# davidbau/rewriting

Hardware: NVIDIA H100
Metric: StyleGAN2-256 images/sec (higher is better)
Workload: dtype bf16x3 (3-term split bf16 operands, fp32 accumulate; fp32 in/out)

## Files before the change

### rewriting_b200/csrc/conv_tc.cu

```cuda
#include <cstdlib>
#include <cstring>

#include "rw_common.cuh"
#include "rw_kernels.h"

namespace rw {

namespace {

constexpr int BM = 128;
constexpr int BK = 32;
constexpr int MMA_K = 16;
constexpr int kStages = 7;
constexpr int kNumThreads = 384;
constexpr int kTmaWarp = 8;
constexpr uint32_t kProducerRegs = 40;
constexpr uint32_t kConsumerRegs = 232;
constexpr int kCluster = 2;
constexpr int kChunkKB = 16;

template <int BN>
struct ConvSmem {
  static constexpr int kABytes = BM * BK * 2;
  static constexpr int kBBytes = BN * BK * 2;
  static constexpr int kStageBytes = 2 * kABytes + 2 * kBBytes;
  static constexpr int kTotal = kStages * kStageBytes + 512  + 256 ;
};
static_assert(ConvSmem<128>::kTotal <= 232448, "conv_tc: shared memory over the per-block limit");

struct Barriers {
  uint64_t full[kStages];
  uint64_t empty[kStages];
};

__device__ __forceinline__ void decode_tile(int tile, int nphase, int nsched, int& ph, int& mn) {
  mn = tile / nphase;
  ph = tile - mn * nphase;
  if (nphase > 1) ph = (ph + ((nsched % nphase) == 0 ? tile / nsched : mn)) % nphase;
}

template <int BN, int EPI, bool PROF>
__global__ void __launch_bounds__(kNumThreads, 1)
conv_tc_kernel(const __grid_constant__ CUtensorMap map_a_hi,
               const __grid_constant__ CUtensorMap map_a_lo,
               const __grid_constant__ CUtensorMap map_w_hi,
               const __grid_constant__ CUtensorMap map_w_lo, const ConvTcParams p) {
  extern __shared__ uint8_t smem_raw[];
  uint8_t* smem = reinterpret_cast<uint8_t*>((reinterpret_cast<uintptr_t>(smem_raw) + 511) &
                                             ~static_cast<uintptr_t>(511));
  using S = ConvSmem<BN>;
  constexpr int NR = BN / 2;
  constexpr int NJ = BN / 8;
  Barriers* bars = reinterpret_cast<Barriers*>(smem + kStages * S::kStageBytes);

  const int warp = __shfl_sync(0xffffffffu, static_cast<int>(threadIdx.x >> 5), 0);
  const int lane = threadIdx.x & 31;
  const int rank = static_cast<int>(cluster_ctarank());
  const int nsched = static_cast<int>(num_clusters_x());
  const int first_unit = static_cast<int>(cluster_id_x());

  const int m_tiles = (p.rows + BM - 1) / BM;
  const int n_tiles = p.Cout / BN;
  const int mn_units = (m_tiles + kCluster - 1) / kCluster * n_tiles;
  const int num_units = mn_units * p.nphase;
  const int kb_per_tap = p.Cin / BK;

  if (warp == kTmaWarp && lane == 0) {
    tma_prefetch_desc(&map_a_hi);
    tma_prefetch_desc(&map_a_lo);
    tma_prefetch_desc(&map_w_hi);
    tma_prefetch_desc(&map_w_lo);
    for (int s = 0; s < kStages; ++s) {
      mbar_init(&bars->full[s], 1);
      mbar_init(&bars->empty[s], 2 * kCluster);
    }
    fence_mbar_init();
  }
  cluster_sync();

  if (warp < kTmaWarp) {
    setmaxnreg_inc<kConsumerRegs>();
    const int wg = threadIdx.x >> 7;
    const int c = lane & 3;
    const int img = p.Hp * p.Wp;
    auto release = [&](int s) {
      if ((threadIdx.x & 127) == 0) {
#pragma unroll
        for (int r = 0; r < kCluster; ++r) mbar_arrive_cluster(mapa_shared(&bars->empty[s], r));
      }
    };
    auto clk = [] { return static_cast<uint32_t>(clock()); };
    uint32_t prof[6] = {0, 0, 0, 0, 0, 0};
    uint32_t tp0 = 0, tp1 = 0;
    if constexpr (PROF) prof[5] = 0u - clk();
    int stage = 0;
    uint32_t phase = 0;
    for (int unit = first_unit; unit < num_units; unit += nsched) {
      int ph, mn;
      decode_tile(unit, p.nphase, nsched, ph, mn);
      const int num_kb = p.ph_ntaps[ph] * kb_per_tap;
      const int n_tile = mn % n_tiles;
      const int n0 = n_tile * BN;
      const int m0 = ((mn / n_tiles) * kCluster + rank) * BM;

      float acc[NR], d[NR];
#pragma unroll
      for (int j = 0; j < NR; ++j) acc[j] = 0.f;
      for (int kb0 = 0; kb0 < num_kb; kb0 += kChunkKB) {
        const int kb_end = (kb0 + kChunkKB < num_kb) ? kb0 + kChunkKB : num_kb;
        int held = -1;
        for (int kb = kb0; kb < kb_end; ++kb) {
          if constexpr (PROF) tp0 = clk();
          mbar_wait(&bars->full[stage], phase);
          if constexpr (PROF) { tp1 = clk(); prof[0] += tp1 - tp0; }
          const uint32_t sa = smem_u32(smem + stage * S::kStageBytes);
          const uint64_t da_hi = make_smem_desc(sa + wg * (S::kABytes / 2), 16, 512, 2);
          const uint64_t da_lo = make_smem_desc(sa + S::kABytes + wg * (S::kABytes / 2), 16, 512, 2);
          const uint64_t db_hi = make_smem_desc(sa + 2 * S::kABytes, 16, 512, 2);
          const uint64_t db_lo = make_smem_desc(sa + 2 * S::kABytes + S::kBBytes, 16, 512, 2);
          wgmma_fence();
#pragma unroll
          for (int kk = 0; kk < BK / MMA_K; ++kk) {
            const uint64_t adv = static_cast<uint64_t>((kk * MMA_K * 2) >> 4);
            wgmma_m64nN<0, 0>(d, da_lo + adv, db_hi + adv, ((kb - kb0) | kk) != 0);
            wgmma_m64nN<0, 0>(d, da_hi + adv, db_lo + adv, 1u);
            wgmma_m64nN<0, 0>(d, da_hi + adv, db_hi + adv, 1u);
          }
          wgmma_commit();
          wgmma_wait<1>();
          if (held >= 0) release(held);
          held = stage;
          if (++stage == kStages) { stage = 0; phase ^= 1u; }
          if constexpr (PROF) prof[1] += clk() - tp1;
        }
        if constexpr (PROF) tp0 = clk();
        wgmma_wait<0>();
        release(held);
#pragma unroll
        for (int j = 0; j < NR; ++j) acc[j] += d[j];
        if constexpr (PROF) prof[2] += clk() - tp0;
      }
      if constexpr (PROF) tp0 = clk();

      uint32_t tid;
      asm volatile("mov.u32 %0, %%tid.x;\n" : "=r"(tid));
      const int row0 = m0 + ((tid >> 7) << 6) + (((tid >> 5) & 3) << 4) + ((tid & 31) >> 2);
#pragma unroll
      for (int i = 0; i < 2; ++i) {
        const int prow = row0 + 8 * i;
        const int b = prow / img;
        const int rem = prow - b * img;
        const int yy = rem / p.Wp;
        const int xx = rem - yy * p.Wp;
        const int Hv = p.ph_Hv[ph], Wv = p.ph_Wv[ph];
        const bool in_rows = prow < p.rows;
        const bool valid = in_rows && (yy < Hv) && (xx < Wv);
        const float* scl = (p.scale_bo && in_rows) ? p.scale_bo + static_cast<size_t>(b) * p.Cout : nullptr;
        float* outp = (p.out != nullptr && p.out_mode == 0 && valid)
                          ? p.out + p.ph_out_ofs[ph] + static_cast<size_t>(b) * p.out_sb +
                                static_cast<size_t>(yy) * p.out_sy + static_cast<size_t>(xx) * p.out_sx
                          : nullptr;
        if (EPI == 1 || !valid) {
          if (scl && (EPI == 1 || p.out_mode == 1)) {
#pragma unroll
            for (int j = 0; j < NJ; ++j) {
              const float2 sv = __ldg(reinterpret_cast<const float2*>(scl + n0 + 8 * j + 2 * c));
              acc[4 * j + 2 * i] *= sv.x;
              acc[4 * j + 2 * i + 1] *= sv.y;
            }
          }
          if (EPI == 1 && outp) {
#pragma unroll
            for (int j = 0; j < NJ; ++j)
#pragma unroll
              for (int e = 0; e < 2; ++e)
                outp[static_cast<size_t>(n0 + 8 * j + 2 * c + e) * p.out_sc] = acc[4 * j + 2 * i + e];
          }
        } else {
          float nz = 0.f;
          if (p.noise != nullptr)
            nz = __ldg(p.noise_w) * __ldg(p.noise + static_cast<size_t>(b) * p.noise_bstride +
                                          static_cast<size_t>(yy) * Wv + xx);
          const float act_gain = p.act_gain != 0.f ? p.act_gain : 1.4142135623730951f;
          if (scl) {
            const float* sc = scl + n0 + 2 * c;
#pragma unroll
            for (int j = 0; j < NJ; ++j)
#pragma unroll
              for (int e = 0; e < 2; ++e) acc[4 * j + 2 * i + e] *= __ldg(sc + 8 * j + e);
          }
#pragma unroll
          for (int j = 0; j < NJ; ++j)
#pragma unroll
            for (int e = 0; e < 2; ++e) acc[4 * j + 2 * i + e] += nz;
          if (p.bias) {
            const float* bi = p.bias + n0 + 2 * c;
#pragma unroll
            for (int j = 0; j < NJ; ++j)
#pragma unroll
              for (int e = 0; e < 2; ++e) acc[4 * j + 2 * i + e] += __ldg(bi + 8 * j + e);
          }
          if (p.act) {
#pragma unroll
            for (int j = 0; j < 2 * NJ; ++j) {
              float& t = acc[4 * (j >> 1) + 2 * i + (j & 1)];
              t = (t > 0.f ? t : 0.2f * t) * act_gain;
            }
          }
          if (outp) {
#pragma unroll
            for (int j = 0; j < NJ; ++j)
#pragma unroll
              for (int e = 0; e < 2; ++e)
                outp[static_cast<size_t>(n0 + 8 * j + 2 * c + e) * p.out_sc] = acc[4 * j + 2 * i + e];
          }
        }
        if (EPI == 0 && p.rgb_w != nullptr) {
          const float* rw0 = p.rgb_w + (static_cast<size_t>(valid ? b : 0) * 3) * p.Cout + n0 + 2 * c;
          const float* rw1 = rw0 + p.Cout;
          const float* rw2 = rw1 + p.Cout;
#pragma unroll
          for (int half = 0; half < BN / 64; ++half) {
            float r0 = 0.f, r1 = 0.f, r2 = 0.f;
            if (valid) {
#pragma unroll
              for (int j = 8 * half; j < 8 * half + 8; ++j)
#pragma unroll
                for (int e = 0; e < 2; ++e) {
                  const float t = acc[4 * j + 2 * i + e];
                  r0 = fmaf(__ldg(rw0 + 8 * j + e), t, r0);
                  r1 = fmaf(__ldg(rw1 + 8 * j + e), t, r1);
                  r2 = fmaf(__ldg(rw2 + 8 * j + e), t, r2);
                }
            }
#pragma unroll
            for (int s = 1; s < 4; s <<= 1) {
              r0 += __shfl_xor_sync(0xffffffffu, r0, s);
              r1 += __shfl_xor_sync(0xffffffffu, r1, s);
              r2 += __shfl_xor_sync(0xffffffffu, r2, s);
            }
            if (valid && c == 0) {
              const size_t hw = static_cast<size_t>(Hv) * Wv;
              float* rp = p.rgb_part + ((static_cast<size_t>(n_tile * (BN / 64) + half) * p.B + b) * 3) * hw +
                          static_cast<size_t>(yy) * Wv + xx;
              rp[0] = r0;
              rp[hw] = r1;
              rp[2 * hw] = r2;
            }
          }
        }
        if (p.out != nullptr && p.out_mode == 1 && in_rows) {
          float* orow = p.out + (static_cast<size_t>(ph) * p.rows + prow) * p.Cout + n0 + 2 * c;
#pragma unroll
          for (int j = 0; j < NJ; ++j)
            *reinterpret_cast<float2*>(orow + 8 * j) = make_float2(acc[4 * j + 2 * i], acc[4 * j + 2 * i + 1]);
        }
        if (EPI == 0 && p.next_hi != nullptr && in_rows) {
          const float* ns = p.next_scale + static_cast<size_t>(valid ? b : 0) * p.Cout + n0 + 2 * c;
          const size_t ofs = static_cast<size_t>(prow) * p.Cout + n0 + 2 * c;
          uint32_t* nh = reinterpret_cast<uint32_t*>(static_cast<__nv_bfloat16*>(p.next_hi) + ofs);
          uint32_t* nl = reinterpret_cast<uint32_t*>(static_cast<__nv_bfloat16*>(p.next_lo) + ofs);
#pragma unroll
          for (int j = 0; j < NJ; ++j) {
            float k0 = 0.f, k1 = 0.f;
            if (valid) {
              const float2 sv = __ldg(reinterpret_cast<const float2*>(ns + 8 * j));
              k0 = sv.x * acc[4 * j + 2 * i];
              k1 = sv.y * acc[4 * j + 2 * i + 1];
            }
            const __nv_bfloat162 hh = __floats2bfloat162_rn(k0, k1);
            const float2 hf = __bfloat1622float2(hh);
            const __nv_bfloat162 ll = __floats2bfloat162_rn(k0 - hf.x, k1 - hf.y);
            nh[4 * j] = *reinterpret_cast<const uint32_t*>(&hh);
            nl[4 * j] = *reinterpret_cast<const uint32_t*>(&ll);
          }
        }
      }
      if constexpr (PROF) { prof[3] += clk() - tp0; prof[4] += 1; }
    }
    if constexpr (PROF) {
      prof[5] += clk();
      if (lane == 0) {
        long long* dst = p.debug_prof + (static_cast<size_t>(blockIdx.x) * 8 + warp) * 8;
#pragma unroll
        for (int i = 0; i < 8; ++i) dst[i] = i < 6 ? prof[i] : 0;
      }
    }
  } else {
    setmaxnreg_dec<kProducerRegs>();
    if (warp == kTmaWarp && lane == 0) {
      constexpr uint16_t kMask = (1u << kCluster) - 1;
      constexpr int kBSlice = BN / kCluster;
      const uint32_t b_off = 2 * S::kABytes + rank * (S::kBBytes / kCluster);
      int stage = 0;
      uint32_t phase = 0;
      for (int unit = first_unit; unit < num_units; unit += nsched) {
        int ph, mn;
        decode_tile(unit, p.nphase, nsched, ph, mn);
        const int n0 = (mn % n_tiles) * BN + rank * kBSlice;
        const int m0 = ((mn / n_tiles) * kCluster + rank) * BM;
        for (int t = 0; t < p.ph_ntaps[ph]; ++t) {
          const int arow = m0 + p.ph_shift[ph][t];
          const int wcol = p.ph_kofs[ph][t];
          const int acol = p.ph_acol[ph][t];
          for (int kb = 0; kb < kb_per_tap; ++kb) {
            mbar_wait(&bars->empty[stage], phase ^ 1u);
            uint8_t* st = smem + stage * S::kStageBytes;
            mbar_expect_tx(&bars->full[stage], S::kStageBytes);
            tma_load_2d(st, &map_a_hi, &bars->full[stage], acol + kb * BK, arow);
            tma_load_2d(st + S::kABytes, &map_a_lo, &bars->full[stage], acol + kb * BK, arow);
            tma_load_2d_multicast(st + b_off, &map_w_hi, &bars->full[stage], wcol + kb * BK, n0,
                                  kMask);
            tma_load_2d_multicast(st + b_off + S::kBBytes, &map_w_lo, &bars->full[stage],
                                  wcol + kb * BK, n0, kMask);
            if (++stage == kStages) { stage = 0; phase ^= 1u; }
          }
        }
      }
    }
    __syncwarp();
  }
  cluster_sync();
}

}

template <int BN, int EPI, bool PROF>
static int conv_tc_launch_epi(const ConvTcParams& p, const void* a_hi, const void* a_lo,
                              const void* w_hi, const void* w_lo, int wk_total,
                              cudaStream_t stream) {
  CUtensorMap ma_hi, ma_lo, mw_hi, mw_lo;
  int rc;
  const uint64_t a_cols = p.a_cols > 0 ? p.a_cols : p.Cin;
  const uint64_t a_dims[2] = {a_cols, static_cast<uint64_t>(p.rows)}, a_str[1] = {a_cols * 2};
  const uint64_t w_dims[2] = {static_cast<uint64_t>(wk_total), static_cast<uint64_t>(p.Cout)};
  const uint64_t w_str[1] = {static_cast<uint64_t>(wk_total) * 2};
  const uint32_t a_box[2] = {BK, BM}, w_box[2] = {BK, BN / kCluster};
  if ((rc = make_tmap_nd_bf16(&ma_hi, a_hi, 2, a_dims, a_str, a_box, nullptr, 3))) return rc;
  if ((rc = make_tmap_nd_bf16(&ma_lo, a_lo, 2, a_dims, a_str, a_box, nullptr, 3))) return rc;
  if ((rc = make_tmap_nd_bf16(&mw_hi, w_hi, 2, w_dims, w_str, w_box, nullptr, 3))) return rc;
  if ((rc = make_tmap_nd_bf16(&mw_lo, w_lo, 2, w_dims, w_str, w_box, nullptr, 3))) return rc;

  cudaLaunchConfig_t cfg = {};
  cudaLaunchAttribute attr[1];
  attr[0].id = cudaLaunchAttributeClusterDimension;
  attr[0].val.clusterDim.x = kCluster;
  attr[0].val.clusterDim.y = 1;
  attr[0].val.clusterDim.z = 1;
  cfg.blockDim = dim3(kNumThreads);
  cfg.dynamicSmemBytes = ConvSmem<BN>::kTotal;
  cfg.stream = stream;
  cfg.attrs = attr;
  cfg.numAttrs = 1;
  static int max_clusters = 0;
  if (max_clusters == 0) {
    rc = check_cuda(cudaFuncSetAttribute(conv_tc_kernel<BN, EPI, PROF>,
                                         cudaFuncAttributeMaxDynamicSharedMemorySize, ConvSmem<BN>::kTotal),
                    "conv_tc smem attr");
    if (rc) return rc;
    cfg.gridDim = dim3(kCluster * (device_sm_count() / kCluster));
    rc = check_cuda(cudaOccupancyMaxActiveClusters(&max_clusters, conv_tc_kernel<BN, EPI, PROF>, &cfg),
                    "conv_tc cluster occupancy");
    if (rc) return rc;
    if (max_clusters < 1) {
      set_last_error("conv_tc: no cluster of %d CTAs fits on the device", kCluster);
      return RW_ERR_UNSUPPORTED;
    }
  }
  const int m_tiles = (p.rows + BM - 1) / BM;
  const int n_tiles = p.Cout / BN;
  const int num_units = (m_tiles + kCluster - 1) / kCluster * n_tiles * p.nphase;
  const int clusters = max_clusters < num_units ? max_clusters : num_units;
  cfg.gridDim = dim3(kCluster * clusters);
  rc = check_cuda(cudaLaunchKernelEx(&cfg, conv_tc_kernel<BN, EPI, PROF>, ma_hi, ma_lo, mw_hi, mw_lo, p),
                  "conv_tc launch");
  if (rc) return rc;
  return check_cuda(cudaGetLastError(), "conv_tc launch");
}

template <int BN>
static int conv_tc_launch_bn(const ConvTcParams& p, const void* a_hi, const void* a_lo,
                             const void* w_hi, const void* w_lo, int wk_total, cudaStream_t stream) {
  const bool lean = !p.noise && !p.bias && !p.act && !p.rgb_w && !p.rgb_part && !p.next_hi &&
                    p.out != nullptr && (reinterpret_cast<uintptr_t>(p.scale_bo) & 7u) == 0;
  if (p.debug_prof) return conv_tc_launch_epi<BN, 0, true>(p, a_hi, a_lo, w_hi, w_lo, wk_total, stream);
  if (lean) return conv_tc_launch_epi<BN, 1, false>(p, a_hi, a_lo, w_hi, w_lo, wk_total, stream);
  return conv_tc_launch_epi<BN, 0, false>(p, a_hi, a_lo, w_hi, w_lo, wk_total, stream);
}

int conv_tc_launch(const ConvTcParams& p, const void* a_hi, const void* a_lo, const void* w_hi,
                   const void* w_lo, int wk_total, cudaStream_t stream) {
  if (p.Cin % 64 != 0 || p.Cout % 64 != 0 || p.nphase < 1 || p.nphase > 4 || p.rows <= 0) {
    set_last_error("conv_tc: unsupported shape Cin=%d Cout=%d nphase=%d rows=%d", p.Cin, p.Cout,
                   p.nphase, p.rows);
    return RW_ERR_BAD_ARG;
  }
  for (int i = 0; i < p.nphase; ++i)
    if (p.ph_ntaps[i] < 1 || p.ph_ntaps[i] > 9) {
      set_last_error("conv_tc: phase %d has %d taps", i, p.ph_ntaps[i]);
      return RW_ERR_BAD_ARG;
    }
  const struct {
    const void* ptr;
    unsigned align;
    const char* name;
  } need[] = {
      {p.scale_bo, p.out_mode == 1 ? 8u : 4u, "scale_bo"},
      {p.out, p.out_mode == 1 ? 8u : 4u, "out"},
      {p.noise, 4u, "noise"},
      {p.noise_w, 4u, "noise_w"},
      {p.bias, 4u, "bias"},
      {p.next_scale, 8u, "next_scale"},
      {p.next_hi, 4u, "next_hi"},
      {p.next_lo, 4u, "next_lo"},
      {p.rgb_w, 4u, "rgb_w"},
      {p.rgb_part, 4u, "rgb_part"},
  };
  for (const auto& n : need)
    if (n.ptr != nullptr && (reinterpret_cast<uintptr_t>(n.ptr) & (n.align - 1)) != 0) {
      set_last_error("conv_tc: %s (%p) is not %u-byte aligned", n.name, n.ptr, n.align);
      return RW_ERR_BAD_ARG;
    }
  if (p.Cout % 128 == 0) return conv_tc_launch_bn<128>(p, a_hi, a_lo, w_hi, w_lo, wk_total, stream);
  return conv_tc_launch_bn<64>(p, a_hi, a_lo, w_hi, w_lo, wk_total, stream);
}

}
```

Baseline: 1976.

## Stage next-layer bf16 hi/lo outputs via stmatrix and TMA bulk stores, add paired-row epilogue

The full epilogue variant now writes the next layer's split bf16 hi/lo activations by packing them into a per-warp shared-memory slot with stmatrix (swizzled) and issuing 2D TMA stores, replacing scattered 32-bit global stores. It also adds a fast path for warps whose two row halves share an image, hoisting the scale, bias and RGB-weight loads across both rows. To make room for the output slots, the pipeline depth for this variant drops from 7 to 6 stages, which may reduce latency hiding in the mainloop. Profiling slots are extended to time the rgb and store phases.

```diff
diff --git a/rewriting_b200/csrc/conv_tc.cu b/rewriting_b200/csrc/conv_tc.cu
--- a/rewriting_b200/csrc/conv_tc.cu
+++ b/rewriting_b200/csrc/conv_tc.cu
@@ -11,7 +11,7 @@
 constexpr int BM = 128;
 constexpr int BK = 32;
 constexpr int MMA_K = 16;
-constexpr int kStages = 7;
+constexpr int kMaxStages = 7;
 constexpr int kNumThreads = 384;
 constexpr int kTmaWarp = 8;
 constexpr uint32_t kProducerRegs = 40;
@@ -19,19 +19,45 @@
 constexpr int kCluster = 2;
 constexpr int kChunkKB = 16;
 
-template <int BN>
+constexpr int kOutSlotBytes = 4096;
+
+template <int BN, int EPI>
 struct ConvSmem {
+  static constexpr int kStages = EPI == 0 ? kMaxStages - 1 : kMaxStages;
   static constexpr int kABytes = BM * BK * 2;
   static constexpr int kBBytes = BN * BK * 2;
   static constexpr int kStageBytes = 2 * kABytes + 2 * kBBytes;
-  static constexpr int kTotal = kStages * kStageBytes + 512  + 256 ;
+  static constexpr int kOutBytes = EPI == 0 ? 8 * kOutSlotBytes : 0;
+  static constexpr int kAlign = EPI == 0 ? 1024 : 512;
+  static constexpr int kTotal = kStages * kStageBytes + kOutBytes + kAlign  +
+                                256 ;
 };
-static_assert(ConvSmem<128>::kTotal <= 232448, "conv_tc: shared memory over the per-block limit");
+static_assert(ConvSmem<128, 0>::kTotal <= 232448, "conv_tc: shared memory over the per-block limit");
+static_assert(ConvSmem<128, 1>::kTotal <= 232448, "conv_tc: shared memory over the per-block limit");
 
 struct Barriers {
-  uint64_t full[kStages];
-  uint64_t empty[kStages];
+  uint64_t full[kMaxStages];
+  uint64_t empty[kMaxStages];
 };
+
+__device__ __forceinline__ void tma_store_2d(const CUtensorMap* m, uint32_t smem_src, int32_t c_inner,
+                                             int32_t c_outer) {
+  asm volatile("cp.async.bulk.tensor.2d.global.shared::cta.bulk_group [%0, {%2, %3}], [%1];\n" ::"l"(
+                   reinterpret_cast<uint64_t>(m)),
+               "r"(smem_src), "r"(c_inner), "r"(c_outer)
+               : "memory");
+}
+__device__ __forceinline__ void bulk_commit() { asm volatile("cp.async.bulk.commit_group;\n" ::: "memory"); }
+__device__ __forceinline__ void bulk_wait_read_all() {
+  asm volatile("cp.async.bulk.wait_group.read 0;\n" ::: "memory");
+}
+__device__ __forceinline__ void bulk_wait_all() { asm volatile("cp.async.bulk.wait_group 0;\n" ::: "memory"); }
+__device__ __forceinline__ void stmatrix_x4(uint32_t addr, uint32_t r0, uint32_t r1, uint32_t r2,
+                                            uint32_t r3) {
+  asm volatile("stmatrix.sync.aligned.m8n8.x4.shared.b16 [%0], {%1, %2, %3, %4};\n" ::"r"(addr),
+               "r"(r0), "r"(r1), "r"(r2), "r"(r3)
+               : "memory");
+}
 
 __device__ __forceinline__ void decode_tile(int tile, int nphase, int nsched, int& ph, int& mn) {
   mn = tile / nphase;
@@ -44,14 +70,17 @@
 conv_tc_kernel(const __grid_constant__ CUtensorMap map_a_hi,
                const __grid_constant__ CUtensorMap map_a_lo,
                const __grid_constant__ CUtensorMap map_w_hi,
-               const __grid_constant__ CUtensorMap map_w_lo, const ConvTcParams p) {
+               const __grid_constant__ CUtensorMap map_w_lo, const ConvTcParams p,
+               const __grid_constant__ CUtensorMap map_n_hi,
+               const __grid_constant__ CUtensorMap map_n_lo) {
+  using S = ConvSmem<BN, EPI>;
+  constexpr int kStages = S::kStages;
   extern __shared__ uint8_t smem_raw[];
-  uint8_t* smem = reinterpret_cast<uint8_t*>((reinterpret_cast<uintptr_t>(smem_raw) + 511) &
-                                             ~static_cast<uintptr_t>(511));
-  using S = ConvSmem<BN>;
+  uint8_t* smem = reinterpret_cast<uint8_t*>((reinterpret_cast<uintptr_t>(smem_raw) + S::kAlign - 1) &
+                                             ~static_cast<uintptr_t>(S::kAlign - 1));
   constexpr int NR = BN / 2;
   constexpr int NJ = BN / 8;
-  Barriers* bars = reinterpret_cast<Barriers*>(smem + kStages * S::kStageBytes);
+  Barriers* bars = reinterpret_cast<Barriers*>(smem + kStages * S::kStageBytes + S::kOutBytes);
 
   const int warp = __shfl_sync(0xffffffffu, static_cast<int>(threadIdx.x >> 5), 0);
   const int lane = threadIdx.x & 31;
@@ -70,6 +99,10 @@
     tma_prefetch_desc(&map_a_lo);
     tma_prefetch_desc(&map_w_hi);
     tma_prefetch_desc(&map_w_lo);
+    if (EPI == 0 && p.next_hi != nullptr) {
+      tma_prefetch_desc(&map_n_hi);
+      tma_prefetch_desc(&map_n_lo);
+    }
     for (int s = 0; s < kStages; ++s) {
       mbar_init(&bars->full[s], 1);
       mbar_init(&bars->empty[s], 2 * kCluster);
@@ -90,7 +123,7 @@
       }
     };
     auto clk = [] { return static_cast<uint32_t>(clock()); };
-    uint32_t prof[6] = {0, 0, 0, 0, 0, 0};
+    uint32_t prof[8] = {0, 0, 0, 0, 0, 0, 0, 0};
     uint32_t tp0 = 0, tp1 = 0;
     if constexpr (PROF) prof[5] = 0u - clk();
     int stage = 0;
@@ -145,6 +178,119 @@
       uint32_t tid;
       asm volatile("mov.u32 %0, %%tid.x;\n" : "=r"(tid));
       const int row0 = m0 + ((tid >> 7) << 6) + (((tid >> 5) & 3) << 4) + ((tid & 31) >> 2);
+      bool row_valid[2];
+      int row_img[2];
+      const bool pair = EPI == 0 && __all_sync(0xffffffffu, row0 + 8 < p.rows &&
+                                                               row0 / img == (row0 + 8) / img) &&
+                        !(p.out != nullptr && p.out_mode == 1);
+      if (pair) {
+        const int b = row0 / img;
+        const int Hv = p.ph_Hv[ph], Wv = p.ph_Wv[ph];
+        int yy[2], xx[2];
+        float nz[2];
+#pragma unroll
+        for (int i = 0; i < 2; ++i) {
+          const int rem = row0 + 8 * i - b * img;
+          yy[i] = rem / p.Wp;
+          xx[i] = rem - yy[i] * p.Wp;
+          row_valid[i] = (yy[i] < Hv) && (xx[i] < Wv);
+          row_img[i] = row_valid[i] ? b : 0;
+          nz[i] = 0.f;
+          if (p.noise != nullptr && row_valid[i])
+            nz[i] = __ldg(p.noise_w) * __ldg(p.noise + static_cast<size_t>(b) * p.noise_bstride +
+                                             static_cast<size_t>(yy[i]) * Wv + xx[i]);
+        }
+        const float act_gain = p.act_gain != 0.f ? p.act_gain : 1.4142135623730951f;
+        if (p.scale_bo) {
+          const float* sc = p.scale_bo + static_cast<size_t>(b) * p.Cout + n0 + 2 * c;
+#pragma unroll
+          for (int j = 0; j < NJ; ++j)
+#pragma unroll
+            for (int e = 0; e < 2; ++e) {
+              const float s = __ldg(sc + 8 * j + e);
+              acc[4 * j + e] *= s;
+              acc[4 * j + 2 + e] *= s;
+            }
+        }
+#pragma unroll
+        for (int j = 0; j < NJ; ++j)
+#pragma unroll
+          for (int e = 0; e < 2; ++e) {
+            acc[4 * j + e] += nz[0];
+            acc[4 * j + 2 + e] += nz[1];
+          }
+        if (p.bias) {
+          const float* bi = p.bias + n0 + 2 * c;
+#pragma unroll
+          for (int j = 0; j < NJ; ++j)
+#pragma unroll
+            for (int e = 0; e < 2; ++e) {
+              const float v = __ldg(bi + 8 * j + e);
+              acc[4 * j + e] += v;
+              acc[4 * j + 2 + e] += v;
+            }
+        }
+        if (p.act) {
+#pragma unroll
+          for (int j = 0; j < NR; ++j) acc[j] = (acc[j] > 0.f ? acc[j] : 0.2f * acc[j]) * act_gain;
+        }
+        if (p.out != nullptr) {
+#pragma unroll
+          for (int i = 0; i < 2; ++i) {
+            if (!row_valid[i]) continue;
+            float* outp = p.out + p.ph_out_ofs[ph] + static_cast<size_t>(b) * p.out_sb +
+                          static_cast<size_t>(yy[i]) * p.out_sy + static_cast<size_t>(xx[i]) * p.out_sx;
+#pragma unroll
+            for (int j = 0; j < NJ; ++j)
+#pragma unroll
+              for (int e = 0; e < 2; ++e)
+                outp[static_cast<size_t>(n0 + 8 * j + 2 * c + e) * p.out_sc] = acc[4 * j + 2 * i + e];
+          }
+        }
+        if (p.rgb_w != nullptr) {
+          if constexpr (PROF) tp1 = clk();
+          const float* rw0 = p.rgb_w + (static_cast<size_t>(b) * 3) * p.Cout + n0 + 2 * c;
+          const float* rw1 = rw0 + p.Cout;
+          const float* rw2 = rw1 + p.Cout;
+#pragma unroll
+          for (int half = 0; half < BN / 64; ++half) {
+            float r[2][3] = {{0.f, 0.f, 0.f}, {0.f, 0.f, 0.f}};
+#pragma unroll
+            for (int j = 8 * half; j < 8 * half + 8; ++j)
+#pragma unroll
+              for (int e = 0; e < 2; ++e) {
+                const float w0 = __ldg(rw0 + 8 * j + e), w1 = __ldg(rw1 + 8 * j + e),
+                            w2 = __ldg(rw2 + 8 * j + e);
+#pragma unroll
+                for (int i = 0; i < 2; ++i) {
+                  const float t = acc[4 * j + 2 * i + e];
+                  r[i][0] = fmaf(w0, t, r[i][0]);
+                  r[i][1] = fmaf(w1, t, r[i][1]);
+                  r[i][2] = fmaf(w2, t, r[i][2]);
+                }
+              }
+#pragma unroll
+            for (int i = 0; i < 2; ++i) {
+#pragma unroll
+              for (int k = 0; k < 3; ++k) r[i][k] = row_valid[i] ? r[i][k] : 0.f;
+#pragma unroll
+              for (int s = 1; s < 4; s <<= 1)
+#pragma unroll
+                for (int k = 0; k < 3; ++k) r[i][k] += __shfl_xor_sync(0xffffffffu, r[i][k], s);
+              if (row_valid[i] && c == 0) {
+                const size_t hw = static_cast<size_t>(Hv) * Wv;
+                float* rp = p.rgb_part + ((static_cast<size_t>(n_tile * (BN / 64) + half) * p.B + b) * 3) * hw +
+                            static_cast<size_t>(yy[i]) * Wv + xx[i];
+                rp[0] = r[i][0];
+                rp[hw] = r[i][1];
+                rp[2 * hw] = r[i][2];
+              }
+            }
+          }
+          if constexpr (PROF) prof[6] += clk() - tp1;
+        }
+      }
+      if (!pair)
 #pragma unroll
       for (int i = 0; i < 2; ++i) {
         const int prow = row0 + 8 * i;
@@ -216,6 +362,7 @@
           }
         }
         if (EPI == 0 && p.rgb_w != nullptr) {
+          if constexpr (PROF) tp1 = clk();
           const float* rw0 = p.rgb_w + (static_cast<size_t>(valid ? b : 0) * 3) * p.Cout + n0 + 2 * c;
           const float* rw1 = rw0 + p.Cout;
           const float* rw2 = rw1 + p.Cout;
@@ -248,6 +395,7 @@
               rp[2 * hw] = r2;
             }
           }
+          if constexpr (PROF) prof[6] += clk() - tp1;
         }
         if (p.out != nullptr && p.out_mode == 1 && in_rows) {
           float* orow = p.out + (static_cast<size_t>(ph) * p.rows + prow) * p.Cout + n0 + 2 * c;
@@ -255,35 +403,65 @@
           for (int j = 0; j < NJ; ++j)
             *reinterpret_cast<float2*>(orow + 8 * j) = make_float2(acc[4 * j + 2 * i], acc[4 * j + 2 * i + 1]);
         }
-        if (EPI == 0 && p.next_hi != nullptr && in_rows) {
-          const float* ns = p.next_scale + static_cast<size_t>(valid ? b : 0) * p.Cout + n0 + 2 * c;
-          const size_t ofs = static_cast<size_t>(prow) * p.Cout + n0 + 2 * c;
-          uint32_t* nh = reinterpret_cast<uint32_t*>(static_cast<__nv_bfloat16*>(p.next_hi) + ofs);
-          uint32_t* nl = reinterpret_cast<uint32_t*>(static_cast<__nv_bfloat16*>(p.next_lo) + ofs);
-#pragma unroll
-          for (int j = 0; j < NJ; ++j) {
-            float k0 = 0.f, k1 = 0.f;
-            if (valid) {
-              const float2 sv = __ldg(reinterpret_cast<const float2*>(ns + 8 * j));
-              k0 = sv.x * acc[4 * j + 2 * i];
-              k1 = sv.y * acc[4 * j + 2 * i + 1];
-            }
-            const __nv_bfloat162 hh = __floats2bfloat162_rn(k0, k1);
-            const float2 hf = __bfloat1622float2(hh);
-            const __nv_bfloat162 ll = __floats2bfloat162_rn(k0 - hf.x, k1 - hf.y);
-            nh[4 * j] = *reinterpret_cast<const uint32_t*>(&hh);
-            nl[4 * j] = *reinterpret_cast<const uint32_t*>(&ll);
-          }
-        }
+        row_valid[i] = valid;
+        row_img[i] = valid ? b : 0;
+      }
+      if (EPI == 0 && p.next_hi != nullptr) {
+        if constexpr (PROF) tp1 = clk();
+        const uint32_t slot = smem_u32(smem + kStages * S::kStageBytes) + warp * kOutSlotBytes;
+        const uint32_t ln = tid & 31;
+        const uint32_t lane_row = slot + ((((ln >> 3) & 1) << 3) + (ln & 7)) * 128;
+        const int warp_row0 = row0 - ((tid & 31) >> 2);
+        const float* ns0 = p.next_scale + static_cast<size_t>(row_img[0]) * p.Cout + n0 + 2 * c;
+        const float* ns1 = p.next_scale + static_cast<size_t>(row_img[1]) * p.Cout + n0 + 2 * c;
+#pragma unroll
+        for (int h = 0; h < BN / 64; ++h) {
+          uint32_t hw[16], lw[16];
+#pragma unroll
+          for (int j = 8 * h; j < 8 * h + 8; ++j)
+#pragma unroll
+            for (int i = 0; i < 2; ++i) {
+              float k0 = 0.f, k1 = 0.f;
+              if (row_valid[i]) {
+                const float2 sv = __ldg(reinterpret_cast<const float2*>((i ? ns1 : ns0) + 8 * j));
+                k0 = sv.x * acc[4 * j + 2 * i];
+                k1 = sv.y * acc[4 * j + 2 * i + 1];
+              }
+              const __nv_bfloat162 hh = __floats2bfloat162_rn(k0, k1);
+              const float2 hf = __bfloat1622float2(hh);
+              const __nv_bfloat162 ll = __floats2bfloat162_rn(k0 - hf.x, k1 - hf.y);
+              hw[2 * (j - 8 * h) + i] = *reinterpret_cast<const uint32_t*>(&hh);
+              lw[2 * (j - 8 * h) + i] = *reinterpret_cast<const uint32_t*>(&ll);
+            }
+          if (ln == 0) bulk_wait_read_all();
+          __syncwarp();
+#pragma unroll
+          for (int q = 0; q < 4; ++q) {
+            const uint32_t a = lane_row + ((((2 * q) | (ln >> 4)) ^ (ln & 7)) << 4);
+            stmatrix_x4(a, hw[4 * q], hw[4 * q + 1], hw[4 * q + 2], hw[4 * q + 3]);
+            stmatrix_x4(a + kOutSlotBytes / 2, lw[4 * q], lw[4 * q + 1], lw[4 * q + 2], lw[4 * q + 3]);
+          }
+          fence_proxy_async_smem();
+          __syncwarp();
+          if (ln == 0) {
+            tma_store_2d(&map_n_hi, slot, n0 + 64 * h, warp_row0);
+            tma_store_2d(&map_n_lo, slot + kOutSlotBytes / 2, n0 + 64 * h, warp_row0);
+            bulk_commit();
+          }
+        }
+        if constexpr (PROF) prof[7] += clk() - tp1;
       }
       if constexpr (PROF) { prof[3] += clk() - tp0; prof[4] += 1; }
     }
+    uint32_t lane_end;
+    asm volatile("mov.u32 %0, %%laneid;\n" : "=r"(lane_end));
+    if (EPI == 0 && p.next_hi != nullptr && lane_end == 0) bulk_wait_all();
     if constexpr (PROF) {
       prof[5] += clk();
-      if (lane == 0) {
+      if (lane_end == 0) {
         long long* dst = p.debug_prof + (static_cast<size_t>(blockIdx.x) * 8 + warp) * 8;
 #pragma unroll
-        for (int i = 0; i < 8; ++i) dst[i] = i < 6 ? prof[i] : 0;
+        for (int i = 0; i < 8; ++i) dst[i] = prof[i];
       }
     }
   } else {
@@ -340,6 +518,17 @@
   if ((rc = make_tmap_nd_bf16(&ma_lo, a_lo, 2, a_dims, a_str, a_box, nullptr, 3))) return rc;
   if ((rc = make_tmap_nd_bf16(&mw_hi, w_hi, 2, w_dims, w_str, w_box, nullptr, 3))) return rc;
   if ((rc = make_tmap_nd_bf16(&mw_lo, w_lo, 2, w_dims, w_str, w_box, nullptr, 3))) return rc;
+  CUtensorMap mn_hi, mn_lo;
+  memset(&mn_hi, 0, sizeof(mn_hi));
+  memset(&mn_lo, 0, sizeof(mn_lo));
+  if (EPI == 0 && p.next_hi != nullptr) {
+    const uint64_t n_dims[2] = {static_cast<uint64_t>(p.Cout), static_cast<uint64_t>(p.rows)};
+    const uint64_t n_str[1] = {static_cast<uint64_t>(p.Cout) * 2};
+    const uint32_t n_box[2] = {64, 16};
+    if ((rc = make_tmap_nd_bf16(&mn_hi, p.next_hi, 2, n_dims, n_str, n_box, nullptr, 2))) return rc;
+    if ((rc = make_tmap_nd_bf16(&mn_lo, p.next_lo, 2, n_dims, n_str, n_box, nullptr, 2))) return rc;
+  }
+  using S = ConvSmem<BN, EPI>;
 
   cudaLaunchConfig_t cfg = {};
   cudaLaunchAttribute attr[1];
@@ -348,14 +537,14 @@
   attr[0].val.clusterDim.y = 1;
   attr[0].val.clusterDim.z = 1;
   cfg.blockDim = dim3(kNumThreads);
-  cfg.dynamicSmemBytes = ConvSmem<BN>::kTotal;
+  cfg.dynamicSmemBytes = S::kTotal;
   cfg.stream = stream;
   cfg.attrs = attr;
   cfg.numAttrs = 1;
   static int max_clusters = 0;
   if (max_clusters == 0) {
     rc = check_cuda(cudaFuncSetAttribute(conv_tc_kernel<BN, EPI, PROF>,
-                                         cudaFuncAttributeMaxDynamicSharedMemorySize, ConvSmem<BN>::kTotal),
+                                         cudaFuncAttributeMaxDynamicSharedMemorySize, S::kTotal),
                     "conv_tc smem attr");
     if (rc) return rc;
     cfg.gridDim = dim3(kCluster * (device_sm_count() / kCluster));
@@ -372,7 +561,8 @@
   const int num_units = (m_tiles + kCluster - 1) / kCluster * n_tiles * p.nphase;
   const int clusters = max_clusters < num_units ? max_clusters : num_units;
   cfg.gridDim = dim3(kCluster * clusters);
-  rc = check_cuda(cudaLaunchKernelEx(&cfg, conv_tc_kernel<BN, EPI, PROF>, ma_hi, ma_lo, mw_hi, mw_lo, p),
+  rc = check_cuda(cudaLaunchKernelEx(&cfg, conv_tc_kernel<BN, EPI, PROF>, ma_hi, ma_lo, mw_hi, mw_lo, p,
+                                     mn_hi, mn_lo),
                   "conv_tc launch");
   if (rc) return rc;
   return check_cuda(cudaGetLastError(), "conv_tc launch");
```

After: 2061 (median of 6 runs). +4.3%, better.
